# Zejun-Yang/AniPortrait

Hardware: NVIDIA H100
Metric: denoised frames/sec @512x512 L=16 steps=25 (higher is better)
Workload: dtype fp16

## Files before the change

aniportrait_b200/csrc/ap_attention.cu:

```cuda
#include <stdio.h>
#include <stdlib.h>

#include "ap_host.h"
#include "ap_ptx.cuh"
#include "ap_wgmma.cuh"

namespace ap {

__device__ __forceinline__ float fast_exp2(float x) {
  float y;
  asm("ex2.approx.ftz.f32 %0, %1;" : "=f"(y) : "f"(x));
  return y;
}

struct AttnParams {
  int n_frames, tokens, heads, head_dim;
  int bank_tokens;
  int first_bank_frame;
  int frames_per_bank;
  int m_tiles;
  int num_units;
  float scale_log2;
  __half* out;
  long long ldo;
};

template <int DPAD, int BN>
struct AttnCfg {
  static constexpr int SLABS = DPAD / 64;
  static constexpr int Q_BYTES = 128 * DPAD * 2;
  static constexpr int K_BYTES = BN * DPAD * 2;
  static constexpr int KV_STAGE = 2 * K_BYTES;
  static constexpr int BUDGET = 227 * 1024 - 1024 - 256 - Q_BYTES;
  static constexpr int STAGES_RAW = BUDGET / KV_STAGE;
  static constexpr int STAGES = STAGES_RAW > 4 ? 4 : STAGES_RAW;
  static constexpr int SMEM_BYTES = Q_BYTES + STAGES * KV_STAGE + 1024 + 256;
  static_assert(STAGES >= 2, "need at least a double-buffered K/V ring");
  static_assert(DPAD % 64 == 0 && DPAD <= 192 && (BN == 64 || BN == 128), "tile config");
};

template <int DPAD, int BN>
__global__ void __launch_bounds__(384, 1)
attention_kernel(const __grid_constant__ CUtensorMap tmQ, const __grid_constant__ CUtensorMap tmK,
                 const __grid_constant__ CUtensorMap tmV, const __grid_constant__ CUtensorMap tmBK,
                 const __grid_constant__ CUtensorMap tmBV, const AttnParams p) {
  using Cfg = AttnCfg<DPAD, BN>;
  constexpr int ST = Cfg::STAGES;
  griddep_launch_dependents();
  extern __shared__ uint8_t smem_raw[];
  uint8_t* smem = reinterpret_cast<uint8_t*>((reinterpret_cast<uintptr_t>(smem_raw) + 1023) & ~uintptr_t(1023));
  uint8_t* smem_q = smem;
  uint8_t* smem_kv = smem_q + Cfg::Q_BYTES;
  uint64_t* bars = reinterpret_cast<uint64_t*>(smem_kv + ST * Cfg::KV_STAGE);
  uint64_t* q_full = bars + 0;
  uint64_t* q_empty = bars + 1;
  uint64_t* k_full = bars + 2;
  uint64_t* v_full = k_full + ST;
  uint64_t* kv_empty = v_full + ST;

  const int warp = threadIdx.x >> 5;
  const int lane = threadIdx.x & 31;

  if (warp == 0 && lane == 0) {
    tma_prefetch_desc(&tmQ);
    tma_prefetch_desc(&tmK);
    tma_prefetch_desc(&tmV);
    mbar_init(q_full, 1);
    mbar_init(q_empty, 8);
    for (int s = 0; s < ST; ++s) {
      mbar_init(&k_full[s], 1);
      mbar_init(&v_full[s], 1);
      mbar_init(&kv_empty[s], 8);
    }
    fence_mbar_init();
  }
  __syncthreads();
  griddep_wait();

  const int own_tiles = (p.tokens + BN - 1) / BN;
  const int bank_tiles = (p.bank_tokens + BN - 1) / BN;
  const int units_per_frame = p.heads * p.m_tiles;

  auto decode = [&](int unit, int& frame, int& head, int& m_tile, int& T) {
    const int fk = unit / units_per_frame;
    const int rem = unit % units_per_frame;
    frame = (fk + p.first_bank_frame) % p.n_frames;
    head = rem / p.m_tiles;
    m_tile = rem % p.m_tiles;
    const bool has_bank = p.bank_tokens > 0 && frame >= p.first_bank_frame;
    T = own_tiles + (has_bank ? bank_tiles : 0);
  };

  if (warp < 4) {
    setmaxnreg_dec<40>();
    if (warp == 0 && lane == 0) {
      uint32_t g = 0;
      uint32_t uc = 0;
      for (int unit = blockIdx.x; unit < p.num_units; unit += gridDim.x, ++uc) {
        int frame, head, m_tile, T;
        decode(unit, frame, head, m_tile, T);
        mbar_wait_quiet(q_empty, (uc & 1) ^ 1);
        mbar_arrive_expect_tx(q_full, Cfg::Q_BYTES);
#pragma unroll
        for (int s = 0; s < Cfg::SLABS; ++s)
          tma_load_2d(&tmQ, q_full, smem_q + s * (128 * 128), head * DPAD + s * 64, frame * p.tokens + m_tile * 128);
        const int bank_idx = (frame - p.first_bank_frame) / p.frames_per_bank;
        for (int j = 0; j < T; ++j, ++g) {
          const int stage = g % ST;
          const uint32_t ph = (g / ST) & 1;
          mbar_wait_quiet(&kv_empty[stage], ph ^ 1);
          const bool own = j < own_tiles;
          const CUtensorMap* mk = own ? &tmK : &tmBK;
          const CUtensorMap* mv = own ? &tmV : &tmBV;
          const int row = own ? frame * p.tokens + j * BN : bank_idx * p.bank_tokens + (j - own_tiles) * BN;
          uint8_t* kd = smem_kv + stage * Cfg::KV_STAGE;
          uint8_t* vd = kd + Cfg::K_BYTES;
          mbar_arrive_expect_tx(&k_full[stage], Cfg::K_BYTES);
#pragma unroll
          for (int s = 0; s < Cfg::SLABS; ++s)
            tma_load_2d(mk, &k_full[stage], kd + s * (BN * 128), head * DPAD + s * 64, row);
          mbar_arrive_expect_tx(&v_full[stage], Cfg::K_BYTES);
#pragma unroll
          for (int s = 0; s < Cfg::SLABS; ++s)
            tma_load_2d(mv, &v_full[stage], vd + s * (BN * 128), head * DPAD + s * 64, row);
        }
      }
    }
    return;
  }

  setmaxnreg_inc<232>();
  const int wg = (warp >> 2) - 1;
  const int wq = warp & 3;
  const int qd = lane & 3;
  const uint32_t q_base = smem_u32(smem_q) + wg * (64 * 128);
  uint32_t g = 0, uc = 0;
  for (int unit = blockIdx.x; unit < p.num_units; unit += gridDim.x, ++uc) {
    int frame, head, m_tile, T;
    decode(unit, frame, head, m_tile, T);
    float o[DPAD / 2];
#pragma unroll
    for (int i = 0; i < DPAD / 2; ++i) o[i] = 0.f;
    float m_run[2] = {-INFINITY, -INFINITY}, l_run[2] = {0.f, 0.f};
    mbar_wait_quiet(q_full, uc & 1);
    for (int j = 0; j < T; ++j, ++g) {
      const int stage = g % ST;
      const uint32_t ph = (g / ST) & 1;
      const uint32_t k_addr = smem_u32(smem_kv + stage * Cfg::KV_STAGE);
      const uint32_t v_addr = k_addr + Cfg::K_BYTES;
      float s[BN / 2];
      mbar_wait_quiet(&k_full[stage], ph);
      wgmma_fence();
#pragma unroll
      for (int kk = 0; kk < DPAD / 16; ++kk)
        wgmma_ss<BN>(s, wgmma_desc_k_sw128(q_base + (kk / 4) * (128 * 128) + (kk % 4) * 32),
                     wgmma_desc_k_sw128(k_addr + (kk / 4) * (BN * 128) + (kk % 4) * 32), kk != 0);
      wgmma_commit();
      wgmma_wait<0>();
      reg_fence<BN / 2>(s);
      if (j == T - 1) {
        __syncwarp();
        if (lane == 0) mbar_arrive(q_empty);
      }

      const bool own = j < own_tiles;
      const int jj = own ? j : j - own_tiles;
      const int ntok = own ? p.tokens : p.bank_tokens;
      const int valid = min(BN, ntok - jj * BN);
      if (valid != BN) {
#pragma unroll
        for (int i = 0; i < BN / 8; ++i)
#pragma unroll
          for (int e = 0; e < 2; ++e)
            if (8 * i + 2 * qd + e >= valid) {
              s[4 * i + e] = -INFINITY;
              s[4 * i + 2 + e] = -INFINITY;
            }
      }
      float mx[2] = {s[0], s[2]};
#pragma unroll
      for (int i = 0; i < BN / 8; ++i) {
        mx[0] = fmaxf(mx[0], fmaxf(s[4 * i], s[4 * i + 1]));
        mx[1] = fmaxf(mx[1], fmaxf(s[4 * i + 2], s[4 * i + 3]));
      }
      float alpha[2];
#pragma unroll
      for (int r = 0; r < 2; ++r) {
        mx[r] = fmaxf(mx[r], __shfl_xor_sync(0xffffffffu, mx[r], 1));
        mx[r] = fmaxf(mx[r], __shfl_xor_sync(0xffffffffu, mx[r], 2));
        const float m_new = fmaxf(m_run[r], mx[r] * p.scale_log2);
        alpha[r] = fast_exp2(m_run[r] - m_new);
        m_run[r] = m_new;
        l_run[r] *= alpha[r];
      }
#pragma unroll
      for (int i = 0; i < DPAD / 8; ++i) {
        o[4 * i] *= alpha[0]; o[4 * i + 1] *= alpha[0];
        o[4 * i + 2] *= alpha[1]; o[4 * i + 3] *= alpha[1];
      }
      uint32_t pk[BN / 4];
#pragma unroll
      for (int i = 0; i < BN / 8; ++i) {
        const float p0 = fast_exp2(fmaf(s[4 * i], p.scale_log2, -m_run[0]));
        const float p1 = fast_exp2(fmaf(s[4 * i + 1], p.scale_log2, -m_run[0]));
        const float p2 = fast_exp2(fmaf(s[4 * i + 2], p.scale_log2, -m_run[1]));
        const float p3 = fast_exp2(fmaf(s[4 * i + 3], p.scale_log2, -m_run[1]));
        l_run[0] += p0 + p1;
        l_run[1] += p2 + p3;
        const __half2 h01 = __floats2half2_rn(p0, p1), h23 = __floats2half2_rn(p2, p3);
        pk[2 * i] = *reinterpret_cast<const uint32_t*>(&h01);
        pk[2 * i + 1] = *reinterpret_cast<const uint32_t*>(&h23);
      }
      mbar_wait_quiet(&v_full[stage], ph);
      wgmma_fence();
#pragma unroll
      for (int kk = 0; kk < BN / 16; ++kk)
        wgmma_rs_tb<DPAD>(o, pk + 4 * kk, wgmma_desc_mn_sw128(v_addr + kk * (16 * 128), BN * 128), 1);
      wgmma_commit();
      wgmma_wait<0>();
      reg_fence<DPAD / 2>(o);
      __syncwarp();
      if (lane == 0) mbar_arrive(&kv_empty[stage]);
    }
#pragma unroll
    for (int r = 0; r < 2; ++r) {
      l_run[r] += __shfl_xor_sync(0xffffffffu, l_run[r], 1);
      l_run[r] += __shfl_xor_sync(0xffffffffu, l_run[r], 2);
    }
#pragma unroll
    for (int r = 0; r < 2; ++r) {
      const float inv_l = 1.f / l_run[r];
      const int q_idx = m_tile * 128 + wg * 64 + wq * 16 + (lane >> 2) + 8 * r;
      if (q_idx < p.tokens) {
        __half* dst = p.out + ((long long)frame * p.tokens + q_idx) * p.ldo + head * p.head_dim;
#pragma unroll
        for (int i = 0; i < DPAD / 8; ++i)
          if (8 * i + 2 * qd < p.head_dim)
            *reinterpret_cast<__half2*>(dst + 8 * i + 2 * qd) =
                __floats2half2_rn(o[4 * i + 2 * r] * inv_l, o[4 * i + 2 * r + 1] * inv_l);
      }
    }
  }
}

template <int DPAD, int BN>
static int launch_attention(const CUtensorMap* maps, const AttnParams& p, cudaStream_t stream) {
  using Cfg = AttnCfg<DPAD, BN>;
  static bool attr_set = false;
  if (!attr_set) {
    AP_CHECK_CUDA(cudaFuncSetAttribute(attention_kernel<DPAD, BN>, cudaFuncAttributeMaxDynamicSharedMemorySize,
                                       Cfg::SMEM_BYTES));
    attr_set = true;
  }
  const int grid = p.num_units < num_sms() ? p.num_units : num_sms();
  AP_LAUNCH((attention_kernel<DPAD, BN>), grid, 384, Cfg::SMEM_BYTES, stream, maps[0], maps[1], maps[2], maps[3], maps[4], p);
  AP_CHECK_CUDA(cudaGetLastError());
  return AP_OK;
}

}

using namespace ap;

extern "C" int ap_attention_f16(const void* q, const void* k, const void* v, long long ld_qkv, const void* bank_k,
                                const void* bank_v, long long ld_bank, int bank_tokens, int n_banks, int n_frames,
                                int tokens, int heads, int head_dim, int dpad, int first_bank_frame,
                                int frames_per_bank, float scale, void* out, long long ldo, void* stream) {
  AP_REQUIRE(q && k && v && out, "attention: null pointer");
  AP_REQUIRE(dpad == 64 || dpad == 128 || dpad == 192, "attention: dpad must be 64/128/192 (got %d)", dpad);
  AP_REQUIRE(head_dim % 8 == 0 && head_dim <= dpad, "attention: head_dim %d must be a multiple of 8 and <= dpad", head_dim);
  AP_REQUIRE(ld_qkv % 8 == 0 && ldo % 8 == 0, "attention: leading dims must be multiples of 8 elements");
  AP_REQUIRE(n_frames > 0 && tokens > 0 && heads > 0, "attention: bad shape");
  const bool has_bank = bank_k != nullptr && bank_tokens > 0;
  AP_REQUIRE(!has_bank || (bank_v && frames_per_bank > 0 && first_bank_frame >= 0 && n_banks > 0),
             "attention: bad bank arguments");
  const int bn = dpad == 192 ? 64 : 128;
  AttnParams p{};
  p.n_frames = n_frames;
  p.tokens = tokens;
  p.heads = heads;
  p.head_dim = head_dim;
  p.bank_tokens = has_bank ? bank_tokens : 0;
  p.first_bank_frame = has_bank ? first_bank_frame : 0;
  p.frames_per_bank = has_bank ? frames_per_bank : 1;
  p.m_tiles = (tokens + 127) / 128;
  p.num_units = n_frames * heads * p.m_tiles;
  p.scale_log2 = scale * 1.4426950408889634f;
  p.out = (__half*)out;
  p.ldo = ldo;
  if (has_bank) {
    const int max_bank = (n_frames - 1 - first_bank_frame) / frames_per_bank;
    AP_REQUIRE(first_bank_frame >= n_frames || max_bank < n_banks, "attention: bank index out of range");
  }

  CUtensorMap maps[5];
  const uint64_t cols = (uint64_t)heads * dpad;
  auto mk = [&](CUtensorMap* tm, const void* base, uint64_t rows, long long ld, uint32_t box_rows) -> int {
    const uint64_t dims[2] = {cols, rows};
    const uint64_t strides[1] = {(uint64_t)ld * 2};
    const uint32_t box[2] = {64, box_rows};
    return encode_tmap(tm, base, 2, dims, strides, box, true);
  };
  int rc;
  const uint64_t rows = (uint64_t)n_frames * tokens;
  if ((rc = mk(&maps[0], q, rows, ld_qkv, 128))) return rc;
  if ((rc = mk(&maps[1], k, rows, ld_qkv, bn))) return rc;
  if ((rc = mk(&maps[2], v, rows, ld_qkv, bn))) return rc;
  if (has_bank) {
    const uint64_t brows = (uint64_t)n_banks * bank_tokens;
    if ((rc = mk(&maps[3], bank_k, brows, ld_bank, bn))) return rc;
    if ((rc = mk(&maps[4], bank_v, brows, ld_bank, bn))) return rc;
  } else {
    maps[3] = maps[1];
    maps[4] = maps[2];
  }
  cudaStream_t st = (cudaStream_t)stream;
  if (dpad == 64) return launch_attention<64, 128>(maps, p, st);
  if (dpad == 128) return launch_attention<128, 128>(maps, p, st);
  return launch_attention<192, 64>(maps, p, st);
}
```

aniportrait_b200/csrc/ap_ptx.cuh:

```cuda
#pragma once
#include <cuda.h>
#include <cuda_fp16.h>
#include <cuda_runtime.h>
#include <stdint.h>
#include <stdio.h>

namespace ap {

__device__ __forceinline__ void griddep_launch_dependents() { asm volatile("griddepcontrol.launch_dependents;" ::: "memory"); }
__device__ __forceinline__ void griddep_wait() { asm volatile("griddepcontrol.wait;" ::: "memory"); }

__device__ __forceinline__ float gelu_erf(float x) {
  const float z = fminf(fabsf(x) * 0.70710678118654752f, 4.3f);
  float q = fmaf(1.686094986e-05f, z, -4.376256625e-04f);
  q = fmaf(q, z, 4.960034474e-03f);
  q = fmaf(q, z, -3.321249048e-02f);
  q = fmaf(q, z, 1.515097036e-01f);
  q = fmaf(q, z, 9.176268788e-01f);
  q = fmaf(q, z, 1.627959694e+00f);
  float e;
  asm("ex2.approx.ftz.f32 %0, %1;" : "=f"(e) : "f"(-q * z));
  return fmaxf(x, 0.f) - z * 0.70710678118654752f * e;
}

__device__ __forceinline__ uint32_t smem_u32(const void* p) {
  return static_cast<uint32_t>(__cvta_generic_to_shared(p));
}

__device__ __forceinline__ uint32_t elect_one() {
  uint32_t pred = 0;
  asm volatile(
      "{\n\t"
      ".reg .pred P1;\n\t"
      "elect.sync _|P1, 0xffffffff;\n\t"
      "selp.u32 %0, 1, 0, P1;\n\t"
      "}\n"
      : "=r"(pred));
  return pred;
}

__device__ __forceinline__ void mbar_init(uint64_t* bar, uint32_t count) {
  asm volatile("mbarrier.init.shared::cta.b64 [%0], %1;" ::"r"(smem_u32(bar)), "r"(count) : "memory");
}
__device__ __forceinline__ void fence_mbar_init() {
  asm volatile("fence.mbarrier_init.release.cluster;" ::: "memory");
}
__device__ __forceinline__ void fence_proxy_async_smem() {
  asm volatile("fence.proxy.async.shared::cta;" ::: "memory");
}
__device__ __forceinline__ void mbar_arrive_expect_tx(uint64_t* bar, uint32_t bytes) {
  asm volatile("mbarrier.arrive.expect_tx.shared::cta.b64 _, [%0], %1;" ::"r"(smem_u32(bar)), "r"(bytes)
               : "memory");
}
__device__ __forceinline__ void mbar_arrive(uint64_t* bar) {
  asm volatile("mbarrier.arrive.shared::cta.b64 _, [%0];" ::"r"(smem_u32(bar)) : "memory");
}
__device__ __forceinline__ uint32_t mbar_try_wait(uint64_t* bar, uint32_t parity) {
  uint32_t done;
  asm volatile(
      "{\n\t"
      ".reg .pred P1;\n\t"
      "mbarrier.try_wait.parity.shared::cta.b64 P1, [%1], %2;\n\t"
      "selp.u32 %0, 1, 0, P1;\n\t"
      "}\n"
      : "=r"(done)
      : "r"(smem_u32(bar)), "r"(parity)
      : "memory");
  return done;
}
#ifndef AP_MBAR_TIMEOUT_CYCLES
#define AP_MBAR_TIMEOUT_CYCLES (8000000000ll)
#endif
__device__ __forceinline__ void mbar_wait(uint64_t* bar, uint32_t parity) {
  if (mbar_try_wait(bar, parity)) return;
  long long t0 = clock64();
  while (!mbar_try_wait(bar, parity)) {
    if (clock64() - t0 > AP_MBAR_TIMEOUT_CYCLES) {
      printf("ap: mbarrier timeout block=(%d,%d) thread=%d bar=0x%x parity=%u\n", blockIdx.x, blockIdx.y, threadIdx.x,
             smem_u32(bar), parity);
      __trap();
    }
  }
}

__device__ __forceinline__ void mbar_wait_quiet(uint64_t* bar, uint32_t parity) {
  if (mbar_try_wait(bar, parity)) return;
  long long t0 = clock64();
  while (!mbar_try_wait(bar, parity))
    if (clock64() - t0 > AP_MBAR_TIMEOUT_CYCLES) __trap();
}

__device__ __forceinline__ void tma_prefetch_desc(const CUtensorMap* m) {
  asm volatile("prefetch.tensormap [%0];" ::"l"(reinterpret_cast<uint64_t>(m)) : "memory");
}
__device__ __forceinline__ void tma_load_2d(const CUtensorMap* m, uint64_t* bar, void* dst, int c0, int c1) {
  asm volatile(
      "cp.async.bulk.tensor.2d.shared::cluster.global.mbarrier::complete_tx::bytes [%0], [%1, {%3, %4}], [%2];" ::"r"(
          smem_u32(dst)),
      "l"(reinterpret_cast<uint64_t>(m)), "r"(smem_u32(bar)), "r"(c0), "r"(c1)
      : "memory");
}
__device__ __forceinline__ void tma_load_3d(const CUtensorMap* m, uint64_t* bar, void* dst, int c0, int c1, int c2) {
  asm volatile(
      "cp.async.bulk.tensor.3d.shared::cluster.global.mbarrier::complete_tx::bytes [%0], [%1, {%3, %4, %5}], [%2];" ::
          "r"(smem_u32(dst)),
      "l"(reinterpret_cast<uint64_t>(m)), "r"(smem_u32(bar)), "r"(c0), "r"(c1), "r"(c2)
      : "memory");
}
__device__ __forceinline__ void tma_load_4d(const CUtensorMap* m, uint64_t* bar, void* dst, int c0, int c1, int c2,
                                            int c3) {
  asm volatile(
      "cp.async.bulk.tensor.4d.shared::cluster.global.mbarrier::complete_tx::bytes [%0], [%1, {%3, %4, %5, %6}], "
      "[%2];" ::"r"(smem_u32(dst)),
      "l"(reinterpret_cast<uint64_t>(m)), "r"(smem_u32(bar)), "r"(c0), "r"(c1), "r"(c2), "r"(c3)
      : "memory");
}
__device__ __forceinline__ void tma_load_5d(const CUtensorMap* m, uint64_t* bar, void* dst, int c0, int c1, int c2,
                                            int c3, int c4) {
  asm volatile(
      "cp.async.bulk.tensor.5d.shared::cluster.global.mbarrier::complete_tx::bytes [%0], [%1, {%3, %4, %5, %6, %7}], "
      "[%2];" ::"r"(smem_u32(dst)),
      "l"(reinterpret_cast<uint64_t>(m)), "r"(smem_u32(bar)), "r"(c0), "r"(c1), "r"(c2), "r"(c3), "r"(c4)
      : "memory");
}

__device__ __forceinline__ void tma_store_2d(const CUtensorMap* m, const void* src, int c0, int c1) {
  asm volatile("cp.async.bulk.tensor.2d.global.shared::cta.bulk_group [%0, {%2, %3}], [%1];" ::"l"(
                   reinterpret_cast<uint64_t>(m)),
               "r"(smem_u32(src)), "r"(c0), "r"(c1)
               : "memory");
}
__device__ __forceinline__ void tma_store_4d(const CUtensorMap* m, const void* src, int c0, int c1, int c2, int c3) {
  asm volatile("cp.async.bulk.tensor.4d.global.shared::cta.bulk_group [%0, {%2, %3, %4, %5}], [%1];" ::"l"(
                   reinterpret_cast<uint64_t>(m)),
               "r"(smem_u32(src)), "r"(c0), "r"(c1), "r"(c2), "r"(c3)
               : "memory");
}
__device__ __forceinline__ void tma_store_commit() { asm volatile("cp.async.bulk.commit_group;" ::: "memory"); }
template <int N>
__device__ __forceinline__ void tma_store_wait_read() {
  asm volatile("cp.async.bulk.wait_group.read %0;" ::"n"(N) : "memory");
}
template <int N>
__device__ __forceinline__ void tma_store_wait_all() {
  asm volatile("cp.async.bulk.wait_group %0;" ::"n"(N) : "memory");
}

__device__ __forceinline__ void wgmma_fence() { asm volatile("wgmma.fence.sync.aligned;" ::: "memory"); }
__device__ __forceinline__ void wgmma_commit() { asm volatile("wgmma.commit_group.sync.aligned;" ::: "memory"); }
template <int N>
__device__ __forceinline__ void wgmma_wait() {
  asm volatile("wgmma.wait_group.sync.aligned %0;" ::"n"(N) : "memory");
}
template <int N>
__device__ __forceinline__ void reg_fence(float* r) {
#pragma unroll
  for (int i = 0; i < N; ++i) asm volatile("" : "+f"(r[i])::"memory");
}
template <uint32_t kRegs>
__device__ __forceinline__ void setmaxnreg_inc() { asm volatile("setmaxnreg.inc.sync.aligned.u32 %0;" ::"n"(kRegs)); }
template <uint32_t kRegs>
__device__ __forceinline__ void setmaxnreg_dec() { asm volatile("setmaxnreg.dec.sync.aligned.u32 %0;" ::"n"(kRegs)); }

__device__ __forceinline__ uint64_t wgmma_desc_k_sw128(uint32_t smem_addr) {
  uint64_t d = 0;
  d |= static_cast<uint64_t>((smem_addr >> 4) & 0x3FFF);
  d |= static_cast<uint64_t>(1) << 16;
  d |= static_cast<uint64_t>(1024 >> 4) << 32;
  d |= static_cast<uint64_t>(1) << 62;
  return d;
}
__device__ __forceinline__ uint64_t wgmma_desc_mn_sw128(uint32_t smem_addr, uint32_t lbo_bytes) {
  uint64_t d = 0;
  d |= static_cast<uint64_t>((smem_addr >> 4) & 0x3FFF);
  d |= static_cast<uint64_t>((lbo_bytes >> 4) & 0x3FFF) << 16;
  d |= static_cast<uint64_t>(1024 >> 4) << 32;
  d |= static_cast<uint64_t>(1) << 62;
  return d;
}

__device__ __forceinline__ void named_bar_sync(uint32_t id, uint32_t nthreads) {
  asm volatile("bar.sync %0, %1;" ::"r"(id), "r"(nthreads) : "memory");
}

}
```

aniportrait_b200/csrc/ap_wgmma.cuh:

```cuda
#pragma once
#include <stdint.h>

namespace ap {

template <int N>
__device__ __forceinline__ void wgmma_ss(float* d, uint64_t da, uint64_t db, uint32_t scale_d);
template <int N>
__device__ __forceinline__ void wgmma_rs_tb(float* d, const uint32_t* a, uint64_t db, uint32_t scale_d);

template <>
__device__ __forceinline__ void wgmma_ss<32>(float* d, uint64_t da, uint64_t db, uint32_t scale_d) {
  asm volatile(
      "{\n\t.reg .pred p;\n\tsetp.ne.b32 p, %18, 0;\n\t"
      "wgmma.mma_async.sync.aligned.m64n32k16.f32.f16.f16 {%0, %1, %2, %3, %4, %5, %6, %7, %8, %9, %10, %11, %12, %13, %14, %15}, %16, %17, p, 1, 1, 0, 0;\n\t}\n"
      : "+f"(d[0]), "+f"(d[1]), "+f"(d[2]), "+f"(d[3]), "+f"(d[4]), "+f"(d[5]), "+f"(d[6]), "+f"(d[7]), "+f"(d[8]), "+f"(d[9]), "+f"(d[10]), "+f"(d[11]), "+f"(d[12]), "+f"(d[13]), "+f"(d[14]), "+f"(d[15])
      : "l"(da), "l"(db), "r"(scale_d));
}
template <>
__device__ __forceinline__ void wgmma_ss<64>(float* d, uint64_t da, uint64_t db, uint32_t scale_d) {
  asm volatile(
      "{\n\t.reg .pred p;\n\tsetp.ne.b32 p, %34, 0;\n\t"
      "wgmma.mma_async.sync.aligned.m64n64k16.f32.f16.f16 {%0, %1, %2, %3, %4, %5, %6, %7, %8, %9, %10, %11, %12, %13, %14, %15, %16, %17, %18, %19, %20, %21, %22, %23, %24, %25, %26, %27, %28, %29, %30, %31}, %32, %33, p, 1, 1, 0, 0;\n\t}\n"
      : "+f"(d[0]), "+f"(d[1]), "+f"(d[2]), "+f"(d[3]), "+f"(d[4]), "+f"(d[5]), "+f"(d[6]), "+f"(d[7]), "+f"(d[8]), "+f"(d[9]), "+f"(d[10]), "+f"(d[11]), "+f"(d[12]), "+f"(d[13]), "+f"(d[14]), "+f"(d[15]), "+f"(d[16]), "+f"(d[17]), "+f"(d[18]), "+f"(d[19]), "+f"(d[20]), "+f"(d[21]), "+f"(d[22]), "+f"(d[23]), "+f"(d[24]), "+f"(d[25]), "+f"(d[26]), "+f"(d[27]), "+f"(d[28]), "+f"(d[29]), "+f"(d[30]), "+f"(d[31])
      : "l"(da), "l"(db), "r"(scale_d));
}
template <>
__device__ __forceinline__ void wgmma_ss<128>(float* d, uint64_t da, uint64_t db, uint32_t scale_d) {
  asm volatile(
      "{\n\t.reg .pred p;\n\tsetp.ne.b32 p, %66, 0;\n\t"
      "wgmma.mma_async.sync.aligned.m64n128k16.f32.f16.f16 {%0, %1, %2, %3, %4, %5, %6, %7, %8, %9, %10, %11, %12, %13, %14, %15, %16, %17, %18, %19, %20, %21, %22, %23, %24, %25, %26, %27, %28, %29, %30, %31, %32, %33, %34, %35, %36, %37, %38, %39, %40, %41, %42, %43, %44, %45, %46, %47, %48, %49, %50, %51, %52, %53, %54, %55, %56, %57, %58, %59, %60, %61, %62, %63}, %64, %65, p, 1, 1, 0, 0;\n\t}\n"
      : "+f"(d[0]), "+f"(d[1]), "+f"(d[2]), "+f"(d[3]), "+f"(d[4]), "+f"(d[5]), "+f"(d[6]), "+f"(d[7]), "+f"(d[8]), "+f"(d[9]), "+f"(d[10]), "+f"(d[11]), "+f"(d[12]), "+f"(d[13]), "+f"(d[14]), "+f"(d[15]), "+f"(d[16]), "+f"(d[17]), "+f"(d[18]), "+f"(d[19]), "+f"(d[20]), "+f"(d[21]), "+f"(d[22]), "+f"(d[23]), "+f"(d[24]), "+f"(d[25]), "+f"(d[26]), "+f"(d[27]), "+f"(d[28]), "+f"(d[29]), "+f"(d[30]), "+f"(d[31]), "+f"(d[32]), "+f"(d[33]), "+f"(d[34]), "+f"(d[35]), "+f"(d[36]), "+f"(d[37]), "+f"(d[38]), "+f"(d[39]), "+f"(d[40]), "+f"(d[41]), "+f"(d[42]), "+f"(d[43]), "+f"(d[44]), "+f"(d[45]), "+f"(d[46]), "+f"(d[47]), "+f"(d[48]), "+f"(d[49]), "+f"(d[50]), "+f"(d[51]), "+f"(d[52]), "+f"(d[53]), "+f"(d[54]), "+f"(d[55]), "+f"(d[56]), "+f"(d[57]), "+f"(d[58]), "+f"(d[59]), "+f"(d[60]), "+f"(d[61]), "+f"(d[62]), "+f"(d[63])
      : "l"(da), "l"(db), "r"(scale_d));
}
template <>
__device__ __forceinline__ void wgmma_ss<160>(float* d, uint64_t da, uint64_t db, uint32_t scale_d) {
  asm volatile(
      "{\n\t.reg .pred p;\n\tsetp.ne.b32 p, %82, 0;\n\t"
      "wgmma.mma_async.sync.aligned.m64n160k16.f32.f16.f16 {%0, %1, %2, %3, %4, %5, %6, %7, %8, %9, %10, %11, %12, %13, %14, %15, %16, %17, %18, %19, %20, %21, %22, %23, %24, %25, %26, %27, %28, %29, %30, %31, %32, %33, %34, %35, %36, %37, %38, %39, %40, %41, %42, %43, %44, %45, %46, %47, %48, %49, %50, %51, %52, %53, %54, %55, %56, %57, %58, %59, %60, %61, %62, %63, %64, %65, %66, %67, %68, %69, %70, %71, %72, %73, %74, %75, %76, %77, %78, %79}, %80, %81, p, 1, 1, 0, 0;\n\t}\n"
      : "+f"(d[0]), "+f"(d[1]), "+f"(d[2]), "+f"(d[3]), "+f"(d[4]), "+f"(d[5]), "+f"(d[6]), "+f"(d[7]), "+f"(d[8]), "+f"(d[9]), "+f"(d[10]), "+f"(d[11]), "+f"(d[12]), "+f"(d[13]), "+f"(d[14]), "+f"(d[15]), "+f"(d[16]), "+f"(d[17]), "+f"(d[18]), "+f"(d[19]), "+f"(d[20]), "+f"(d[21]), "+f"(d[22]), "+f"(d[23]), "+f"(d[24]), "+f"(d[25]), "+f"(d[26]), "+f"(d[27]), "+f"(d[28]), "+f"(d[29]), "+f"(d[30]), "+f"(d[31]), "+f"(d[32]), "+f"(d[33]), "+f"(d[34]), "+f"(d[35]), "+f"(d[36]), "+f"(d[37]), "+f"(d[38]), "+f"(d[39]), "+f"(d[40]), "+f"(d[41]), "+f"(d[42]), "+f"(d[43]), "+f"(d[44]), "+f"(d[45]), "+f"(d[46]), "+f"(d[47]), "+f"(d[48]), "+f"(d[49]), "+f"(d[50]), "+f"(d[51]), "+f"(d[52]), "+f"(d[53]), "+f"(d[54]), "+f"(d[55]), "+f"(d[56]), "+f"(d[57]), "+f"(d[58]), "+f"(d[59]), "+f"(d[60]), "+f"(d[61]), "+f"(d[62]), "+f"(d[63]), "+f"(d[64]), "+f"(d[65]), "+f"(d[66]), "+f"(d[67]), "+f"(d[68]), "+f"(d[69]), "+f"(d[70]), "+f"(d[71]), "+f"(d[72]), "+f"(d[73]), "+f"(d[74]), "+f"(d[75]), "+f"(d[76]), "+f"(d[77]), "+f"(d[78]), "+f"(d[79])
      : "l"(da), "l"(db), "r"(scale_d));
}
template <>
__device__ __forceinline__ void wgmma_ss<256>(float* d, uint64_t da, uint64_t db, uint32_t scale_d) {
  asm volatile(
      "{\n\t.reg .pred p;\n\tsetp.ne.b32 p, %130, 0;\n\t"
      "wgmma.mma_async.sync.aligned.m64n256k16.f32.f16.f16 {%0, %1, %2, %3, %4, %5, %6, %7, %8, %9, %10, %11, %12, %13, %14, %15, %16, %17, %18, %19, %20, %21, %22, %23, %24, %25, %26, %27, %28, %29, %30, %31, %32, %33, %34, %35, %36, %37, %38, %39, %40, %41, %42, %43, %44, %45, %46, %47, %48, %49, %50, %51, %52, %53, %54, %55, %56, %57, %58, %59, %60, %61, %62, %63, %64, %65, %66, %67, %68, %69, %70, %71, %72, %73, %74, %75, %76, %77, %78, %79, %80, %81, %82, %83, %84, %85, %86, %87, %88, %89, %90, %91, %92, %93, %94, %95, %96, %97, %98, %99, %100, %101, %102, %103, %104, %105, %106, %107, %108, %109, %110, %111, %112, %113, %114, %115, %116, %117, %118, %119, %120, %121, %122, %123, %124, %125, %126, %127}, %128, %129, p, 1, 1, 0, 0;\n\t}\n"
      : "+f"(d[0]), "+f"(d[1]), "+f"(d[2]), "+f"(d[3]), "+f"(d[4]), "+f"(d[5]), "+f"(d[6]), "+f"(d[7]), "+f"(d[8]), "+f"(d[9]), "+f"(d[10]), "+f"(d[11]), "+f"(d[12]), "+f"(d[13]), "+f"(d[14]), "+f"(d[15]), "+f"(d[16]), "+f"(d[17]), "+f"(d[18]), "+f"(d[19]), "+f"(d[20]), "+f"(d[21]), "+f"(d[22]), "+f"(d[23]), "+f"(d[24]), "+f"(d[25]), "+f"(d[26]), "+f"(d[27]), "+f"(d[28]), "+f"(d[29]), "+f"(d[30]), "+f"(d[31]), "+f"(d[32]), "+f"(d[33]), "+f"(d[34]), "+f"(d[35]), "+f"(d[36]), "+f"(d[37]), "+f"(d[38]), "+f"(d[39]), "+f"(d[40]), "+f"(d[41]), "+f"(d[42]), "+f"(d[43]), "+f"(d[44]), "+f"(d[45]), "+f"(d[46]), "+f"(d[47]), "+f"(d[48]), "+f"(d[49]), "+f"(d[50]), "+f"(d[51]), "+f"(d[52]), "+f"(d[53]), "+f"(d[54]), "+f"(d[55]), "+f"(d[56]), "+f"(d[57]), "+f"(d[58]), "+f"(d[59]), "+f"(d[60]), "+f"(d[61]), "+f"(d[62]), "+f"(d[63]), "+f"(d[64]), "+f"(d[65]), "+f"(d[66]), "+f"(d[67]), "+f"(d[68]), "+f"(d[69]), "+f"(d[70]), "+f"(d[71]), "+f"(d[72]), "+f"(d[73]), "+f"(d[74]), "+f"(d[75]), "+f"(d[76]), "+f"(d[77]), "+f"(d[78]), "+f"(d[79]), "+f"(d[80]), "+f"(d[81]), "+f"(d[82]), "+f"(d[83]), "+f"(d[84]), "+f"(d[85]), "+f"(d[86]), "+f"(d[87]), "+f"(d[88]), "+f"(d[89]), "+f"(d[90]), "+f"(d[91]), "+f"(d[92]), "+f"(d[93]), "+f"(d[94]), "+f"(d[95]), "+f"(d[96]), "+f"(d[97]), "+f"(d[98]), "+f"(d[99]), "+f"(d[100]), "+f"(d[101]), "+f"(d[102]), "+f"(d[103]), "+f"(d[104]), "+f"(d[105]), "+f"(d[106]), "+f"(d[107]), "+f"(d[108]), "+f"(d[109]), "+f"(d[110]), "+f"(d[111]), "+f"(d[112]), "+f"(d[113]), "+f"(d[114]), "+f"(d[115]), "+f"(d[116]), "+f"(d[117]), "+f"(d[118]), "+f"(d[119]), "+f"(d[120]), "+f"(d[121]), "+f"(d[122]), "+f"(d[123]), "+f"(d[124]), "+f"(d[125]), "+f"(d[126]), "+f"(d[127])
      : "l"(da), "l"(db), "r"(scale_d));
}
template <>
__device__ __forceinline__ void wgmma_rs_tb<64>(float* d, const uint32_t* a, uint64_t db, uint32_t scale_d) {
  asm volatile(
      "{\n\t.reg .pred p;\n\tsetp.ne.b32 p, %37, 0;\n\t"
      "wgmma.mma_async.sync.aligned.m64n64k16.f32.f16.f16 {%0, %1, %2, %3, %4, %5, %6, %7, %8, %9, %10, %11, %12, %13, %14, %15, %16, %17, %18, %19, %20, %21, %22, %23, %24, %25, %26, %27, %28, %29, %30, %31}, {%32, %33, %34, %35}, %36, p, 1, 1, 1;\n\t}\n"
      : "+f"(d[0]), "+f"(d[1]), "+f"(d[2]), "+f"(d[3]), "+f"(d[4]), "+f"(d[5]), "+f"(d[6]), "+f"(d[7]), "+f"(d[8]), "+f"(d[9]), "+f"(d[10]), "+f"(d[11]), "+f"(d[12]), "+f"(d[13]), "+f"(d[14]), "+f"(d[15]), "+f"(d[16]), "+f"(d[17]), "+f"(d[18]), "+f"(d[19]), "+f"(d[20]), "+f"(d[21]), "+f"(d[22]), "+f"(d[23]), "+f"(d[24]), "+f"(d[25]), "+f"(d[26]), "+f"(d[27]), "+f"(d[28]), "+f"(d[29]), "+f"(d[30]), "+f"(d[31])
      : "r"(a[0]), "r"(a[1]), "r"(a[2]), "r"(a[3]), "l"(db), "r"(scale_d));
}
template <>
__device__ __forceinline__ void wgmma_rs_tb<128>(float* d, const uint32_t* a, uint64_t db, uint32_t scale_d) {
  asm volatile(
      "{\n\t.reg .pred p;\n\tsetp.ne.b32 p, %69, 0;\n\t"
      "wgmma.mma_async.sync.aligned.m64n128k16.f32.f16.f16 {%0, %1, %2, %3, %4, %5, %6, %7, %8, %9, %10, %11, %12, %13, %14, %15, %16, %17, %18, %19, %20, %21, %22, %23, %24, %25, %26, %27, %28, %29, %30, %31, %32, %33, %34, %35, %36, %37, %38, %39, %40, %41, %42, %43, %44, %45, %46, %47, %48, %49, %50, %51, %52, %53, %54, %55, %56, %57, %58, %59, %60, %61, %62, %63}, {%64, %65, %66, %67}, %68, p, 1, 1, 1;\n\t}\n"
      : "+f"(d[0]), "+f"(d[1]), "+f"(d[2]), "+f"(d[3]), "+f"(d[4]), "+f"(d[5]), "+f"(d[6]), "+f"(d[7]), "+f"(d[8]), "+f"(d[9]), "+f"(d[10]), "+f"(d[11]), "+f"(d[12]), "+f"(d[13]), "+f"(d[14]), "+f"(d[15]), "+f"(d[16]), "+f"(d[17]), "+f"(d[18]), "+f"(d[19]), "+f"(d[20]), "+f"(d[21]), "+f"(d[22]), "+f"(d[23]), "+f"(d[24]), "+f"(d[25]), "+f"(d[26]), "+f"(d[27]), "+f"(d[28]), "+f"(d[29]), "+f"(d[30]), "+f"(d[31]), "+f"(d[32]), "+f"(d[33]), "+f"(d[34]), "+f"(d[35]), "+f"(d[36]), "+f"(d[37]), "+f"(d[38]), "+f"(d[39]), "+f"(d[40]), "+f"(d[41]), "+f"(d[42]), "+f"(d[43]), "+f"(d[44]), "+f"(d[45]), "+f"(d[46]), "+f"(d[47]), "+f"(d[48]), "+f"(d[49]), "+f"(d[50]), "+f"(d[51]), "+f"(d[52]), "+f"(d[53]), "+f"(d[54]), "+f"(d[55]), "+f"(d[56]), "+f"(d[57]), "+f"(d[58]), "+f"(d[59]), "+f"(d[60]), "+f"(d[61]), "+f"(d[62]), "+f"(d[63])
      : "r"(a[0]), "r"(a[1]), "r"(a[2]), "r"(a[3]), "l"(db), "r"(scale_d));
}
template <>
__device__ __forceinline__ void wgmma_rs_tb<192>(float* d, const uint32_t* a, uint64_t db, uint32_t scale_d) {
  asm volatile(
      "{\n\t.reg .pred p;\n\tsetp.ne.b32 p, %101, 0;\n\t"
      "wgmma.mma_async.sync.aligned.m64n192k16.f32.f16.f16 {%0, %1, %2, %3, %4, %5, %6, %7, %8, %9, %10, %11, %12, %13, %14, %15, %16, %17, %18, %19, %20, %21, %22, %23, %24, %25, %26, %27, %28, %29, %30, %31, %32, %33, %34, %35, %36, %37, %38, %39, %40, %41, %42, %43, %44, %45, %46, %47, %48, %49, %50, %51, %52, %53, %54, %55, %56, %57, %58, %59, %60, %61, %62, %63, %64, %65, %66, %67, %68, %69, %70, %71, %72, %73, %74, %75, %76, %77, %78, %79, %80, %81, %82, %83, %84, %85, %86, %87, %88, %89, %90, %91, %92, %93, %94, %95}, {%96, %97, %98, %99}, %100, p, 1, 1, 1;\n\t}\n"
      : "+f"(d[0]), "+f"(d[1]), "+f"(d[2]), "+f"(d[3]), "+f"(d[4]), "+f"(d[5]), "+f"(d[6]), "+f"(d[7]), "+f"(d[8]), "+f"(d[9]), "+f"(d[10]), "+f"(d[11]), "+f"(d[12]), "+f"(d[13]), "+f"(d[14]), "+f"(d[15]), "+f"(d[16]), "+f"(d[17]), "+f"(d[18]), "+f"(d[19]), "+f"(d[20]), "+f"(d[21]), "+f"(d[22]), "+f"(d[23]), "+f"(d[24]), "+f"(d[25]), "+f"(d[26]), "+f"(d[27]), "+f"(d[28]), "+f"(d[29]), "+f"(d[30]), "+f"(d[31]), "+f"(d[32]), "+f"(d[33]), "+f"(d[34]), "+f"(d[35]), "+f"(d[36]), "+f"(d[37]), "+f"(d[38]), "+f"(d[39]), "+f"(d[40]), "+f"(d[41]), "+f"(d[42]), "+f"(d[43]), "+f"(d[44]), "+f"(d[45]), "+f"(d[46]), "+f"(d[47]), "+f"(d[48]), "+f"(d[49]), "+f"(d[50]), "+f"(d[51]), "+f"(d[52]), "+f"(d[53]), "+f"(d[54]), "+f"(d[55]), "+f"(d[56]), "+f"(d[57]), "+f"(d[58]), "+f"(d[59]), "+f"(d[60]), "+f"(d[61]), "+f"(d[62]), "+f"(d[63]), "+f"(d[64]), "+f"(d[65]), "+f"(d[66]), "+f"(d[67]), "+f"(d[68]), "+f"(d[69]), "+f"(d[70]), "+f"(d[71]), "+f"(d[72]), "+f"(d[73]), "+f"(d[74]), "+f"(d[75]), "+f"(d[76]), "+f"(d[77]), "+f"(d[78]), "+f"(d[79]), "+f"(d[80]), "+f"(d[81]), "+f"(d[82]), "+f"(d[83]), "+f"(d[84]), "+f"(d[85]), "+f"(d[86]), "+f"(d[87]), "+f"(d[88]), "+f"(d[89]), "+f"(d[90]), "+f"(d[91]), "+f"(d[92]), "+f"(d[93]), "+f"(d[94]), "+f"(d[95])
      : "r"(a[0]), "r"(a[1]), "r"(a[2]), "r"(a[3]), "l"(db), "r"(scale_d));
}

}
```

Measured before the change: 5.601.

## Pipeline QK/PV wgmma in attention, add 3-consumer mode and exact head-dim tiles

Restructures the attention consumer loop so the QK^T wgmma for tile j is issued together with the PV wgmma for tile j-1, overlapping softmax with tensor-core work. For small head dims it uses three consumer warpgroups (192-row Q tiles) with rebalanced register allocation. The kernel is now templated on the head dim rounded up to 16 rather than padded to 64, which cuts wasted MMA work. It also computes some exponentials with a cubic polynomial on FMA units to offload the MUFU unit. Risks include register pressure with the extra live accumulators, lower polynomial precision, and more template instantiations.

After: 5.766, median of 6. 2.9% higher.

```diff
diff --git a/aniportrait_b200/csrc/ap_attention.cu b/aniportrait_b200/csrc/ap_attention.cu
--- a/aniportrait_b200/csrc/ap_attention.cu
+++ b/aniportrait_b200/csrc/ap_attention.cu
@@ -15,6 +15,7 @@
 
 struct AttnParams {
   int n_frames, tokens, heads, head_dim;
+  int dpad;
   int bank_tokens;
   int first_bank_frame;
   int frames_per_bank;
@@ -25,10 +26,26 @@
   long long ldo;
 };
 
-template <int DPAD, int BN>
+#ifndef AP_ATTN_POLY_OF_16
+#define AP_ATTN_POLY_OF_16 2
+#endif
+constexpr int POLY_OF_16 = AP_ATTN_POLY_OF_16;
+
+template <int DH>
+struct AttnKeyTile {
+  static constexpr int value = DH > 128 ? 64 : 128;
+};
+
+#ifndef AP_ATTN_NC3_MAX_DH
+#define AP_ATTN_NC3_MAX_DH 64
+#endif
+__host__ __device__ constexpr int attn_consumers(int dh) { return dh <= AP_ATTN_NC3_MAX_DH ? 3 : 2; }
+
+template <int DPAD, int BN, int NC>
 struct AttnCfg {
   static constexpr int SLABS = DPAD / 64;
-  static constexpr int Q_BYTES = 128 * DPAD * 2;
+  static constexpr int Q_ROWS = 64 * NC;
+  static constexpr int Q_BYTES = Q_ROWS * DPAD * 2;
   static constexpr int K_BYTES = BN * DPAD * 2;
   static constexpr int KV_STAGE = 2 * K_BYTES;
   static constexpr int BUDGET = 227 * 1024 - 1024 - 256 - Q_BYTES;
@@ -39,12 +56,16 @@
   static_assert(DPAD % 64 == 0 && DPAD <= 192 && (BN == 64 || BN == 128), "tile config");
 };
 
-template <int DPAD, int BN>
-__global__ void __launch_bounds__(384, 1)
+template <int DH>
+__global__ void __launch_bounds__(128 * (1 + attn_consumers(DH)), 1)
 attention_kernel(const __grid_constant__ CUtensorMap tmQ, const __grid_constant__ CUtensorMap tmK,
                  const __grid_constant__ CUtensorMap tmV, const __grid_constant__ CUtensorMap tmBK,
                  const __grid_constant__ CUtensorMap tmBV, const AttnParams p) {
-  using Cfg = AttnCfg<DPAD, BN>;
+  constexpr int DPAD = (DH + 63) / 64 * 64;
+  constexpr int BN = AttnKeyTile<DH>::value;
+  constexpr int NC = attn_consumers(DH);
+  using Cfg = AttnCfg<DPAD, BN, NC>;
+  static_assert(DH % 16 == 0, "head dim step");
   constexpr int ST = Cfg::STAGES;
   griddep_launch_dependents();
   extern __shared__ uint8_t smem_raw[];
@@ -66,11 +87,11 @@
     tma_prefetch_desc(&tmK);
     tma_prefetch_desc(&tmV);
     mbar_init(q_full, 1);
-    mbar_init(q_empty, 8);
+    mbar_init(q_empty, 4 * NC);
     for (int s = 0; s < ST; ++s) {
       mbar_init(&k_full[s], 1);
       mbar_init(&v_full[s], 1);
-      mbar_init(&kv_empty[s], 8);
+      mbar_init(&kv_empty[s], 4 * NC);
     }
     fence_mbar_init();
   }
@@ -92,7 +113,7 @@
   };
 
   if (warp < 4) {
-    setmaxnreg_dec<40>();
+    setmaxnreg_dec<NC == 3 ? 24 : 40>();
     if (warp == 0 && lane == 0) {
       uint32_t g = 0;
       uint32_t uc = 0;
@@ -103,7 +124,8 @@
         mbar_arrive_expect_tx(q_full, Cfg::Q_BYTES);
 #pragma unroll
         for (int s = 0; s < Cfg::SLABS; ++s)
-          tma_load_2d(&tmQ, q_full, smem_q + s * (128 * 128), head * DPAD + s * 64, frame * p.tokens + m_tile * 128);
+          tma_load_2d(&tmQ, q_full, smem_q + s * (Cfg::Q_ROWS * 128), head * p.dpad + s * 64,
+                      frame * p.tokens + m_tile * Cfg::Q_ROWS);
         const int bank_idx = (frame - p.first_bank_frame) / p.frames_per_bank;
         for (int j = 0; j < T; ++j, ++g) {
           const int stage = g % ST;
@@ -118,110 +140,149 @@
           mbar_arrive_expect_tx(&k_full[stage], Cfg::K_BYTES);
 #pragma unroll
           for (int s = 0; s < Cfg::SLABS; ++s)
-            tma_load_2d(mk, &k_full[stage], kd + s * (BN * 128), head * DPAD + s * 64, row);
+            tma_load_2d(mk, &k_full[stage], kd + s * (BN * 128), head * p.dpad + s * 64, row);
           mbar_arrive_expect_tx(&v_full[stage], Cfg::K_BYTES);
 #pragma unroll
           for (int s = 0; s < Cfg::SLABS; ++s)
-            tma_load_2d(mv, &v_full[stage], vd + s * (BN * 128), head * DPAD + s * 64, row);
+            tma_load_2d(mv, &v_full[stage], vd + s * (BN * 128), head * p.dpad + s * 64, row);
         }
       }
     }
     return;
   }
 
-  setmaxnreg_inc<232>();
+  setmaxnreg_inc<NC == 3 ? 160 : 232>();
   const int wg = (warp >> 2) - 1;
   const int wq = warp & 3;
   const int qd = lane & 3;
   const uint32_t q_base = smem_u32(smem_q) + wg * (64 * 128);
+
+  auto k_smem = [&](uint32_t t) { return smem_u32(smem_kv + (t % ST) * Cfg::KV_STAGE); };
+  auto issue_qk = [&](float* s, uint32_t k_addr) {
+#pragma unroll
+    for (int kk = 0; kk < DH / 16; ++kk)
+      wgmma_ss<BN>(s, wgmma_desc_k_sw128(q_base + (kk / 4) * (Cfg::Q_ROWS * 128) + (kk % 4) * 32),
+                   wgmma_desc_k_sw128(k_addr + (kk / 4) * (BN * 128) + (kk % 4) * 32), kk != 0);
+  };
+  auto issue_pv = [&](float* o, const uint32_t* pk, uint32_t v_addr) {
+#pragma unroll
+    for (int kk = 0; kk < BN / 16; ++kk)
+      wgmma_rs_tb<DH>(o, pk + 4 * kk, wgmma_desc_mn_sw128(v_addr + kk * (16 * 128), BN * 128), 1);
+  };
+  auto softmax = [&](float* s, int j, int own_tiles, float* m_run, float* l_run, float* alpha) {
+    const bool own = j < own_tiles;
+    const int jj = own ? j : j - own_tiles;
+    const int ntok = own ? p.tokens : p.bank_tokens;
+    const int valid = min(BN, ntok - jj * BN);
+    if (valid != BN) {
+#pragma unroll
+      for (int i = 0; i < BN / 8; ++i)
+#pragma unroll
+        for (int e = 0; e < 2; ++e)
+          if (8 * i + 2 * qd + e >= valid) {
+            s[4 * i + e] = -INFINITY;
+            s[4 * i + 2 + e] = -INFINITY;
+          }
+    }
+    float mx[2] = {s[0], s[2]};
+#pragma unroll
+    for (int i = 0; i < BN / 8; ++i) {
+      mx[0] = fmaxf(mx[0], fmaxf(s[4 * i], s[4 * i + 1]));
+      mx[1] = fmaxf(mx[1], fmaxf(s[4 * i + 2], s[4 * i + 3]));
+    }
+#pragma unroll
+    for (int r = 0; r < 2; ++r) {
+      mx[r] = fmaxf(mx[r], __shfl_xor_sync(0xffffffffu, mx[r], 1));
+      mx[r] = fmaxf(mx[r], __shfl_xor_sync(0xffffffffu, mx[r], 2));
+      const float m_new = fmaxf(m_run[r], mx[r] * p.scale_log2);
+      alpha[r] = fast_exp2(m_run[r] - m_new);
+      m_run[r] = m_new;
+      l_run[r] *= alpha[r];
+    }
+#pragma unroll
+    for (int i = 0; i < BN / 8; ++i) {
+#pragma unroll
+      for (int e = 0; e < 4; ++e) {
+        const float x = fmaf(s[4 * i + e], p.scale_log2, -m_run[e >> 1]);
+        s[4 * i + e] = (4 * i + e) % 16 < POLY_OF_16 ? exp2_poly3(x) : fast_exp2(x);
+      }
+      l_run[0] += s[4 * i] + s[4 * i + 1];
+      l_run[1] += s[4 * i + 2] + s[4 * i + 3];
+    }
+  };
+  auto pack = [&](const float* s, uint32_t* pk) {
+#pragma unroll
+    for (int i = 0; i < BN / 8; ++i) {
+      const __half2 h01 = __floats2half2_rn(s[4 * i], s[4 * i + 1]), h23 = __floats2half2_rn(s[4 * i + 2], s[4 * i + 3]);
+      pk[2 * i] = *reinterpret_cast<const uint32_t*>(&h01);
+      pk[2 * i + 1] = *reinterpret_cast<const uint32_t*>(&h23);
+    }
+  };
+  auto release_q = [&]() {
+    __syncwarp();
+    if (lane == 0) mbar_arrive(q_empty);
+  };
+  auto release_kv = [&](uint32_t t) {
+    __syncwarp();
+    if (lane == 0) mbar_arrive(&kv_empty[t % ST]);
+  };
+
   uint32_t g = 0, uc = 0;
   for (int unit = blockIdx.x; unit < p.num_units; unit += gridDim.x, ++uc) {
     int frame, head, m_tile, T;
     decode(unit, frame, head, m_tile, T);
-    float o[DPAD / 2];
-#pragma unroll
-    for (int i = 0; i < DPAD / 2; ++i) o[i] = 0.f;
-    float m_run[2] = {-INFINITY, -INFINITY}, l_run[2] = {0.f, 0.f};
+    float o[DH / 2];
+#pragma unroll
+    for (int i = 0; i < DH / 2; ++i) o[i] = 0.f;
+    float m_run[2] = {-INFINITY, -INFINITY}, l_run[2] = {0.f, 0.f}, alpha[2];
+    float s[BN / 2];
+    uint32_t pk[BN / 4];
     mbar_wait_quiet(q_full, uc & 1);
-    for (int j = 0; j < T; ++j, ++g) {
-      const int stage = g % ST;
-      const uint32_t ph = (g / ST) & 1;
-      const uint32_t k_addr = smem_u32(smem_kv + stage * Cfg::KV_STAGE);
-      const uint32_t v_addr = k_addr + Cfg::K_BYTES;
-      float s[BN / 2];
-      mbar_wait_quiet(&k_full[stage], ph);
+
+    mbar_wait_quiet(&k_full[g % ST], (g / ST) & 1);
+    wgmma_fence();
+    issue_qk(s, k_smem(g));
+    wgmma_commit();
+    wgmma_wait<0>();
+    reg_fence<BN / 2>(s);
+    if (T == 1) release_q();
+    softmax(s, 0, own_tiles, m_run, l_run, alpha);
+    pack(s, pk);
+
+    for (int j = 1; j < T; ++j) {
+      const uint32_t t = g + j;
+      mbar_wait_quiet(&k_full[t % ST], (t / ST) & 1);
+      mbar_wait_quiet(&v_full[(t - 1) % ST], ((t - 1) / ST) & 1);
       wgmma_fence();
-#pragma unroll
-      for (int kk = 0; kk < DPAD / 16; ++kk)
-        wgmma_ss<BN>(s, wgmma_desc_k_sw128(q_base + (kk / 4) * (128 * 128) + (kk % 4) * 32),
-                     wgmma_desc_k_sw128(k_addr + (kk / 4) * (BN * 128) + (kk % 4) * 32), kk != 0);
+      issue_qk(s, k_smem(t));
       wgmma_commit();
+      issue_pv(o, pk, k_smem(t - 1) + Cfg::K_BYTES);
+      wgmma_commit();
+      wgmma_wait<1>();
+      reg_fence<BN / 2>(s);
+      if (j == T - 1) release_q();
+      softmax(s, j, own_tiles, m_run, l_run, alpha);
       wgmma_wait<0>();
+      reg_fence<DH / 2>(o);
       reg_fence<BN / 2>(s);
-      if (j == T - 1) {
-        __syncwarp();
-        if (lane == 0) mbar_arrive(q_empty);
-      }
-
-      const bool own = j < own_tiles;
-      const int jj = own ? j : j - own_tiles;
-      const int ntok = own ? p.tokens : p.bank_tokens;
-      const int valid = min(BN, ntok - jj * BN);
-      if (valid != BN) {
-#pragma unroll
-        for (int i = 0; i < BN / 8; ++i)
-#pragma unroll
-          for (int e = 0; e < 2; ++e)
-            if (8 * i + 2 * qd + e >= valid) {
-              s[4 * i + e] = -INFINITY;
-              s[4 * i + 2 + e] = -INFINITY;
-            }
-      }
-      float mx[2] = {s[0], s[2]};
-#pragma unroll
-      for (int i = 0; i < BN / 8; ++i) {
-        mx[0] = fmaxf(mx[0], fmaxf(s[4 * i], s[4 * i + 1]));
-        mx[1] = fmaxf(mx[1], fmaxf(s[4 * i + 2], s[4 * i + 3]));
-      }
-      float alpha[2];
-#pragma unroll
-      for (int r = 0; r < 2; ++r) {
-        mx[r] = fmaxf(mx[r], __shfl_xor_sync(0xffffffffu, mx[r], 1));
-        mx[r] = fmaxf(mx[r], __shfl_xor_sync(0xffffffffu, mx[r], 2));
-        const float m_new = fmaxf(m_run[r], mx[r] * p.scale_log2);
-        alpha[r] = fast_exp2(m_run[r] - m_new);
-        m_run[r] = m_new;
-        l_run[r] *= alpha[r];
-      }
-#pragma unroll
-      for (int i = 0; i < DPAD / 8; ++i) {
+      release_kv(t - 1);
+#pragma unroll
+      for (int i = 0; i < DH / 8; ++i) {
         o[4 * i] *= alpha[0]; o[4 * i + 1] *= alpha[0];
         o[4 * i + 2] *= alpha[1]; o[4 * i + 3] *= alpha[1];
       }
-      uint32_t pk[BN / 4];
-#pragma unroll
-      for (int i = 0; i < BN / 8; ++i) {
-        const float p0 = fast_exp2(fmaf(s[4 * i], p.scale_log2, -m_run[0]));
-        const float p1 = fast_exp2(fmaf(s[4 * i + 1], p.scale_log2, -m_run[0]));
-        const float p2 = fast_exp2(fmaf(s[4 * i + 2], p.scale_log2, -m_run[1]));
-        const float p3 = fast_exp2(fmaf(s[4 * i + 3], p.scale_log2, -m_run[1]));
-        l_run[0] += p0 + p1;
-        l_run[1] += p2 + p3;
-        const __half2 h01 = __floats2half2_rn(p0, p1), h23 = __floats2half2_rn(p2, p3);
-        pk[2 * i] = *reinterpret_cast<const uint32_t*>(&h01);
-        pk[2 * i + 1] = *reinterpret_cast<const uint32_t*>(&h23);
-      }
-      mbar_wait_quiet(&v_full[stage], ph);
-      wgmma_fence();
-#pragma unroll
-      for (int kk = 0; kk < BN / 16; ++kk)
-        wgmma_rs_tb<DPAD>(o, pk + 4 * kk, wgmma_desc_mn_sw128(v_addr + kk * (16 * 128), BN * 128), 1);
-      wgmma_commit();
-      wgmma_wait<0>();
-      reg_fence<DPAD / 2>(o);
-      __syncwarp();
-      if (lane == 0) mbar_arrive(&kv_empty[stage]);
-    }
+      pack(s, pk);
+    }
+    const uint32_t t_last = g + T - 1;
+    mbar_wait_quiet(&v_full[t_last % ST], (t_last / ST) & 1);
+    wgmma_fence();
+    issue_pv(o, pk, k_smem(t_last) + Cfg::K_BYTES);
+    wgmma_commit();
+    wgmma_wait<0>();
+    reg_fence<DH / 2>(o);
+    release_kv(t_last);
+    g += T;
+
 #pragma unroll
     for (int r = 0; r < 2; ++r) {
       l_run[r] += __shfl_xor_sync(0xffffffffu, l_run[r], 1);
@@ -230,11 +291,11 @@
 #pragma unroll
     for (int r = 0; r < 2; ++r) {
       const float inv_l = 1.f / l_run[r];
-      const int q_idx = m_tile * 128 + wg * 64 + wq * 16 + (lane >> 2) + 8 * r;
+      const int q_idx = m_tile * Cfg::Q_ROWS + wg * 64 + wq * 16 + (lane >> 2) + 8 * r;
       if (q_idx < p.tokens) {
         __half* dst = p.out + ((long long)frame * p.tokens + q_idx) * p.ldo + head * p.head_dim;
 #pragma unroll
-        for (int i = 0; i < DPAD / 8; ++i)
+        for (int i = 0; i < DH / 8; ++i)
           if (8 * i + 2 * qd < p.head_dim)
             *reinterpret_cast<__half2*>(dst + 8 * i + 2 * qd) =
                 __floats2half2_rn(o[4 * i + 2 * r] * inv_l, o[4 * i + 2 * r + 1] * inv_l);
@@ -243,17 +304,18 @@
   }
 }
 
-template <int DPAD, int BN>
+template <int DH>
 static int launch_attention(const CUtensorMap* maps, const AttnParams& p, cudaStream_t stream) {
-  using Cfg = AttnCfg<DPAD, BN>;
+  using Cfg = AttnCfg<(DH + 63) / 64 * 64, AttnKeyTile<DH>::value, attn_consumers(DH)>;
   static bool attr_set = false;
   if (!attr_set) {
-    AP_CHECK_CUDA(cudaFuncSetAttribute(attention_kernel<DPAD, BN>, cudaFuncAttributeMaxDynamicSharedMemorySize,
+    AP_CHECK_CUDA(cudaFuncSetAttribute(attention_kernel<DH>, cudaFuncAttributeMaxDynamicSharedMemorySize,
                                        Cfg::SMEM_BYTES));
     attr_set = true;
   }
   const int grid = p.num_units < num_sms() ? p.num_units : num_sms();
-  AP_LAUNCH((attention_kernel<DPAD, BN>), grid, 384, Cfg::SMEM_BYTES, stream, maps[0], maps[1], maps[2], maps[3], maps[4], p);
+  AP_LAUNCH((attention_kernel<DH>), grid, 128 * (1 + attn_consumers(DH)), Cfg::SMEM_BYTES, stream, maps[0], maps[1], maps[2], maps[3],
+            maps[4], p);
   AP_CHECK_CUDA(cudaGetLastError());
   return AP_OK;
 }
@@ -274,16 +336,19 @@
   const bool has_bank = bank_k != nullptr && bank_tokens > 0;
   AP_REQUIRE(!has_bank || (bank_v && frames_per_bank > 0 && first_bank_frame >= 0 && n_banks > 0),
              "attention: bad bank arguments");
-  const int bn = dpad == 192 ? 64 : 128;
+  const int dh = (head_dim + 15) / 16 * 16;
+  const int bn = dh > 128 ? 64 : 128;
   AttnParams p{};
   p.n_frames = n_frames;
   p.tokens = tokens;
   p.heads = heads;
   p.head_dim = head_dim;
+  p.dpad = dpad;
   p.bank_tokens = has_bank ? bank_tokens : 0;
   p.first_bank_frame = has_bank ? first_bank_frame : 0;
   p.frames_per_bank = has_bank ? frames_per_bank : 1;
-  p.m_tiles = (tokens + 127) / 128;
+  const int q_rows = 64 * attn_consumers(dh);
+  p.m_tiles = (tokens + q_rows - 1) / q_rows;
   p.num_units = n_frames * heads * p.m_tiles;
   p.scale_log2 = scale * 1.4426950408889634f;
   p.out = (__half*)out;
@@ -303,7 +368,7 @@
   };
   int rc;
   const uint64_t rows = (uint64_t)n_frames * tokens;
-  if ((rc = mk(&maps[0], q, rows, ld_qkv, 128))) return rc;
+  if ((rc = mk(&maps[0], q, rows, ld_qkv, q_rows))) return rc;
   if ((rc = mk(&maps[1], k, rows, ld_qkv, bn))) return rc;
   if ((rc = mk(&maps[2], v, rows, ld_qkv, bn))) return rc;
   if (has_bank) {
@@ -315,7 +380,18 @@
     maps[4] = maps[2];
   }
   cudaStream_t st = (cudaStream_t)stream;
-  if (dpad == 64) return launch_attention<64, 128>(maps, p, st);
-  if (dpad == 128) return launch_attention<128, 128>(maps, p, st);
-  return launch_attention<192, 64>(maps, p, st);
-}
+  switch (dh / 16) {
+    case 1: return launch_attention<16>(maps, p, st);
+    case 2: return launch_attention<32>(maps, p, st);
+    case 3: return launch_attention<48>(maps, p, st);
+    case 4: return launch_attention<64>(maps, p, st);
+    case 5: return launch_attention<80>(maps, p, st);
+    case 6: return launch_attention<96>(maps, p, st);
+    case 7: return launch_attention<112>(maps, p, st);
+    case 8: return launch_attention<128>(maps, p, st);
+    case 9: return launch_attention<144>(maps, p, st);
+    case 10: return launch_attention<160>(maps, p, st);
+    case 11: return launch_attention<176>(maps, p, st);
+    default: return launch_attention<192>(maps, p, st);
+  }
+}
diff --git a/aniportrait_b200/csrc/ap_ptx.cuh b/aniportrait_b200/csrc/ap_ptx.cuh
--- a/aniportrait_b200/csrc/ap_ptx.cuh
+++ b/aniportrait_b200/csrc/ap_ptx.cuh
@@ -21,6 +21,19 @@
   float e;
   asm("ex2.approx.ftz.f32 %0, %1;" : "=f"(e) : "f"(-q * z));
   return fmaxf(x, 0.f) - z * 0.70710678118654752f * e;
+}
+
+__device__ __forceinline__ float exp2_poly3(float x) {
+  x = fmaxf(x, -127.f);
+  const float j = x + 12582912.f;
+  const float f = x - (j - 12582912.f);
+  float p = fmaf(5.517167031e-02f, f, 2.426111252e-01f);
+  p = fmaf(p, f, 6.932609853e-01f);
+  p = fmaf(p, f, 9.999280730e-01f);
+  const float scale = __uint_as_float((__float_as_uint(j) << 23) + 0x3F800000u);
+  float r;
+  asm("mul.ftz.f32 %0, %1, %2;" : "=f"(r) : "f"(p), "f"(scale));
+  return r;
 }
 
 __device__ __forceinline__ uint32_t smem_u32(const void* p) {
diff --git a/aniportrait_b200/csrc/ap_wgmma.cuh b/aniportrait_b200/csrc/ap_wgmma.cuh
--- a/aniportrait_b200/csrc/ap_wgmma.cuh
+++ b/aniportrait_b200/csrc/ap_wgmma.cuh
@@ -49,6 +49,30 @@
       : "l"(da), "l"(db), "r"(scale_d));
 }
 template <>
+__device__ __forceinline__ void wgmma_rs_tb<16>(float* d, const uint32_t* a, uint64_t db, uint32_t scale_d) {
+  asm volatile(
+      "{\n\t.reg .pred p;\n\tsetp.ne.b32 p, %13, 0;\n\t"
+      "wgmma.mma_async.sync.aligned.m64n16k16.f32.f16.f16 {%0, %1, %2, %3, %4, %5, %6, %7}, {%8, %9, %10, %11}, %12, p, 1, 1, 1;\n\t}\n"
+      : "+f"(d[0]), "+f"(d[1]), "+f"(d[2]), "+f"(d[3]), "+f"(d[4]), "+f"(d[5]), "+f"(d[6]), "+f"(d[7])
+      : "r"(a[0]), "r"(a[1]), "r"(a[2]), "r"(a[3]), "l"(db), "r"(scale_d));
+}
+template <>
+__device__ __forceinline__ void wgmma_rs_tb<32>(float* d, const uint32_t* a, uint64_t db, uint32_t scale_d) {
+  asm volatile(
+      "{\n\t.reg .pred p;\n\tsetp.ne.b32 p, %21, 0;\n\t"
+      "wgmma.mma_async.sync.aligned.m64n32k16.f32.f16.f16 {%0, %1, %2, %3, %4, %5, %6, %7, %8, %9, %10, %11, %12, %13, %14, %15}, {%16, %17, %18, %19}, %20, p, 1, 1, 1;\n\t}\n"
+      : "+f"(d[0]), "+f"(d[1]), "+f"(d[2]), "+f"(d[3]), "+f"(d[4]), "+f"(d[5]), "+f"(d[6]), "+f"(d[7]), "+f"(d[8]), "+f"(d[9]), "+f"(d[10]), "+f"(d[11]), "+f"(d[12]), "+f"(d[13]), "+f"(d[14]), "+f"(d[15])
+      : "r"(a[0]), "r"(a[1]), "r"(a[2]), "r"(a[3]), "l"(db), "r"(scale_d));
+}
+template <>
+__device__ __forceinline__ void wgmma_rs_tb<48>(float* d, const uint32_t* a, uint64_t db, uint32_t scale_d) {
+  asm volatile(
+      "{\n\t.reg .pred p;\n\tsetp.ne.b32 p, %29, 0;\n\t"
+      "wgmma.mma_async.sync.aligned.m64n48k16.f32.f16.f16 {%0, %1, %2, %3, %4, %5, %6, %7, %8, %9, %10, %11, %12, %13, %14, %15, %16, %17, %18, %19, %20, %21, %22, %23}, {%24, %25, %26, %27}, %28, p, 1, 1, 1;\n\t}\n"
+      : "+f"(d[0]), "+f"(d[1]), "+f"(d[2]), "+f"(d[3]), "+f"(d[4]), "+f"(d[5]), "+f"(d[6]), "+f"(d[7]), "+f"(d[8]), "+f"(d[9]), "+f"(d[10]), "+f"(d[11]), "+f"(d[12]), "+f"(d[13]), "+f"(d[14]), "+f"(d[15]), "+f"(d[16]), "+f"(d[17]), "+f"(d[18]), "+f"(d[19]), "+f"(d[20]), "+f"(d[21]), "+f"(d[22]), "+f"(d[23])
+      : "r"(a[0]), "r"(a[1]), "r"(a[2]), "r"(a[3]), "l"(db), "r"(scale_d));
+}
+template <>
 __device__ __forceinline__ void wgmma_rs_tb<64>(float* d, const uint32_t* a, uint64_t db, uint32_t scale_d) {
   asm volatile(
       "{\n\t.reg .pred p;\n\tsetp.ne.b32 p, %37, 0;\n\t"
@@ -57,11 +81,59 @@
       : "r"(a[0]), "r"(a[1]), "r"(a[2]), "r"(a[3]), "l"(db), "r"(scale_d));
 }
 template <>
+__device__ __forceinline__ void wgmma_rs_tb<80>(float* d, const uint32_t* a, uint64_t db, uint32_t scale_d) {
+  asm volatile(
+      "{\n\t.reg .pred p;\n\tsetp.ne.b32 p, %45, 0;\n\t"
+      "wgmma.mma_async.sync.aligned.m64n80k16.f32.f16.f16 {%0, %1, %2, %3, %4, %5, %6, %7, %8, %9, %10, %11, %12, %13, %14, %15, %16, %17, %18, %19, %20, %21, %22, %23, %24, %25, %26, %27, %28, %29, %30, %31, %32, %33, %34, %35, %36, %37, %38, %39}, {%40, %41, %42, %43}, %44, p, 1, 1, 1;\n\t}\n"
+      : "+f"(d[0]), "+f"(d[1]), "+f"(d[2]), "+f"(d[3]), "+f"(d[4]), "+f"(d[5]), "+f"(d[6]), "+f"(d[7]), "+f"(d[8]), "+f"(d[9]), "+f"(d[10]), "+f"(d[11]), "+f"(d[12]), "+f"(d[13]), "+f"(d[14]), "+f"(d[15]), "+f"(d[16]), "+f"(d[17]), "+f"(d[18]), "+f"(d[19]), "+f"(d[20]), "+f"(d[21]), "+f"(d[22]), "+f"(d[23]), "+f"(d[24]), "+f"(d[25]), "+f"(d[26]), "+f"(d[27]), "+f"(d[28]), "+f"(d[29]), "+f"(d[30]), "+f"(d[31]), "+f"(d[32]), "+f"(d[33]), "+f"(d[34]), "+f"(d[35]), "+f"(d[36]), "+f"(d[37]), "+f"(d[38]), "+f"(d[39])
+      : "r"(a[0]), "r"(a[1]), "r"(a[2]), "r"(a[3]), "l"(db), "r"(scale_d));
+}
+template <>
+__device__ __forceinline__ void wgmma_rs_tb<96>(float* d, const uint32_t* a, uint64_t db, uint32_t scale_d) {
+  asm volatile(
+      "{\n\t.reg .pred p;\n\tsetp.ne.b32 p, %53, 0;\n\t"
+      "wgmma.mma_async.sync.aligned.m64n96k16.f32.f16.f16 {%0, %1, %2, %3, %4, %5, %6, %7, %8, %9, %10, %11, %12, %13, %14, %15, %16, %17, %18, %19, %20, %21, %22, %23, %24, %25, %26, %27, %28, %29, %30, %31, %32, %33, %34, %35, %36, %37, %38, %39, %40, %41, %42, %43, %44, %45, %46, %47}, {%48, %49, %50, %51}, %52, p, 1, 1, 1;\n\t}\n"
+      : "+f"(d[0]), "+f"(d[1]), "+f"(d[2]), "+f"(d[3]), "+f"(d[4]), "+f"(d[5]), "+f"(d[6]), "+f"(d[7]), "+f"(d[8]), "+f"(d[9]), "+f"(d[10]), "+f"(d[11]), "+f"(d[12]), "+f"(d[13]), "+f"(d[14]), "+f"(d[15]), "+f"(d[16]), "+f"(d[17]), "+f"(d[18]), "+f"(d[19]), "+f"(d[20]), "+f"(d[21]), "+f"(d[22]), "+f"(d[23]), "+f"(d[24]), "+f"(d[25]), "+f"(d[26]), "+f"(d[27]), "+f"(d[28]), "+f"(d[29]), "+f"(d[30]), "+f"(d[31]), "+f"(d[32]), "+f"(d[33]), "+f"(d[34]), "+f"(d[35]), "+f"(d[36]), "+f"(d[37]), "+f"(d[38]), "+f"(d[39]), "+f"(d[40]), "+f"(d[41]), "+f"(d[42]), "+f"(d[43]), "+f"(d[44]), "+f"(d[45]), "+f"(d[46]), "+f"(d[47])
+      : "r"(a[0]), "r"(a[1]), "r"(a[2]), "r"(a[3]), "l"(db), "r"(scale_d));
+}
+template <>
+__device__ __forceinline__ void wgmma_rs_tb<112>(float* d, const uint32_t* a, uint64_t db, uint32_t scale_d) {
+  asm volatile(
+      "{\n\t.reg .pred p;\n\tsetp.ne.b32 p, %61, 0;\n\t"
+      "wgmma.mma_async.sync.aligned.m64n112k16.f32.f16.f16 {%0, %1, %2, %3, %4, %5, %6, %7, %8, %9, %10, %11, %12, %13, %14, %15, %16, %17, %18, %19, %20, %21, %22, %23, %24, %25, %26, %27, %28, %29, %30, %31, %32, %33, %34, %35, %36, %37, %38, %39, %40, %41, %42, %43, %44, %45, %46, %47, %48, %49, %50, %51, %52, %53, %54, %55}, {%56, %57, %58, %59}, %60, p, 1, 1, 1;\n\t}\n"
+      : "+f"(d[0]), "+f"(d[1]), "+f"(d[2]), "+f"(d[3]), "+f"(d[4]), "+f"(d[5]), "+f"(d[6]), "+f"(d[7]), "+f"(d[8]), "+f"(d[9]), "+f"(d[10]), "+f"(d[11]), "+f"(d[12]), "+f"(d[13]), "+f"(d[14]), "+f"(d[15]), "+f"(d[16]), "+f"(d[17]), "+f"(d[18]), "+f"(d[19]), "+f"(d[20]), "+f"(d[21]), "+f"(d[22]), "+f"(d[23]), "+f"(d[24]), "+f"(d[25]), "+f"(d[26]), "+f"(d[27]), "+f"(d[28]), "+f"(d[29]), "+f"(d[30]), "+f"(d[31]), "+f"(d[32]), "+f"(d[33]), "+f"(d[34]), "+f"(d[35]), "+f"(d[36]), "+f"(d[37]), "+f"(d[38]), "+f"(d[39]), "+f"(d[40]), "+f"(d[41]), "+f"(d[42]), "+f"(d[43]), "+f"(d[44]), "+f"(d[45]), "+f"(d[46]), "+f"(d[47]), "+f"(d[48]), "+f"(d[49]), "+f"(d[50]), "+f"(d[51]), "+f"(d[52]), "+f"(d[53]), "+f"(d[54]), "+f"(d[55])
+      : "r"(a[0]), "r"(a[1]), "r"(a[2]), "r"(a[3]), "l"(db), "r"(scale_d));
+}
+template <>
 __device__ __forceinline__ void wgmma_rs_tb<128>(float* d, const uint32_t* a, uint64_t db, uint32_t scale_d) {
   asm volatile(
       "{\n\t.reg .pred p;\n\tsetp.ne.b32 p, %69, 0;\n\t"
       "wgmma.mma_async.sync.aligned.m64n128k16.f32.f16.f16 {%0, %1, %2, %3, %4, %5, %6, %7, %8, %9, %10, %11, %12, %13, %14, %15, %16, %17, %18, %19, %20, %21, %22, %23, %24, %25, %26, %27, %28, %29, %30, %31, %32, %33, %34, %35, %36, %37, %38, %39, %40, %41, %42, %43, %44, %45, %46, %47, %48, %49, %50, %51, %52, %53, %54, %55, %56, %57, %58, %59, %60, %61, %62, %63}, {%64, %65, %66, %67}, %68, p, 1, 1, 1;\n\t}\n"
       : "+f"(d[0]), "+f"(d[1]), "+f"(d[2]), "+f"(d[3]), "+f"(d[4]), "+f"(d[5]), "+f"(d[6]), "+f"(d[7]), "+f"(d[8]), "+f"(d[9]), "+f"(d[10]), "+f"(d[11]), "+f"(d[12]), "+f"(d[13]), "+f"(d[14]), "+f"(d[15]), "+f"(d[16]), "+f"(d[17]), "+f"(d[18]), "+f"(d[19]), "+f"(d[20]), "+f"(d[21]), "+f"(d[22]), "+f"(d[23]), "+f"(d[24]), "+f"(d[25]), "+f"(d[26]), "+f"(d[27]), "+f"(d[28]), "+f"(d[29]), "+f"(d[30]), "+f"(d[31]), "+f"(d[32]), "+f"(d[33]), "+f"(d[34]), "+f"(d[35]), "+f"(d[36]), "+f"(d[37]), "+f"(d[38]), "+f"(d[39]), "+f"(d[40]), "+f"(d[41]), "+f"(d[42]), "+f"(d[43]), "+f"(d[44]), "+f"(d[45]), "+f"(d[46]), "+f"(d[47]), "+f"(d[48]), "+f"(d[49]), "+f"(d[50]), "+f"(d[51]), "+f"(d[52]), "+f"(d[53]), "+f"(d[54]), "+f"(d[55]), "+f"(d[56]), "+f"(d[57]), "+f"(d[58]), "+f"(d[59]), "+f"(d[60]), "+f"(d[61]), "+f"(d[62]), "+f"(d[63])
+      : "r"(a[0]), "r"(a[1]), "r"(a[2]), "r"(a[3]), "l"(db), "r"(scale_d));
+}
+template <>
+__device__ __forceinline__ void wgmma_rs_tb<144>(float* d, const uint32_t* a, uint64_t db, uint32_t scale_d) {
+  asm volatile(
+      "{\n\t.reg .pred p;\n\tsetp.ne.b32 p, %77, 0;\n\t"
+      "wgmma.mma_async.sync.aligned.m64n144k16.f32.f16.f16 {%0, %1, %2, %3, %4, %5, %6, %7, %8, %9, %10, %11, %12, %13, %14, %15, %16, %17, %18, %19, %20, %21, %22, %23, %24, %25, %26, %27, %28, %29, %30, %31, %32, %33, %34, %35, %36, %37, %38, %39, %40, %41, %42, %43, %44, %45, %46, %47, %48, %49, %50, %51, %52, %53, %54, %55, %56, %57, %58, %59, %60, %61, %62, %63, %64, %65, %66, %67, %68, %69, %70, %71}, {%72, %73, %74, %75}, %76, p, 1, 1, 1;\n\t}\n"
+      : "+f"(d[0]), "+f"(d[1]), "+f"(d[2]), "+f"(d[3]), "+f"(d[4]), "+f"(d[5]), "+f"(d[6]), "+f"(d[7]), "+f"(d[8]), "+f"(d[9]), "+f"(d[10]), "+f"(d[11]), "+f"(d[12]), "+f"(d[13]), "+f"(d[14]), "+f"(d[15]), "+f"(d[16]), "+f"(d[17]), "+f"(d[18]), "+f"(d[19]), "+f"(d[20]), "+f"(d[21]), "+f"(d[22]), "+f"(d[23]), "+f"(d[24]), "+f"(d[25]), "+f"(d[26]), "+f"(d[27]), "+f"(d[28]), "+f"(d[29]), "+f"(d[30]), "+f"(d[31]), "+f"(d[32]), "+f"(d[33]), "+f"(d[34]), "+f"(d[35]), "+f"(d[36]), "+f"(d[37]), "+f"(d[38]), "+f"(d[39]), "+f"(d[40]), "+f"(d[41]), "+f"(d[42]), "+f"(d[43]), "+f"(d[44]), "+f"(d[45]), "+f"(d[46]), "+f"(d[47]), "+f"(d[48]), "+f"(d[49]), "+f"(d[50]), "+f"(d[51]), "+f"(d[52]), "+f"(d[53]), "+f"(d[54]), "+f"(d[55]), "+f"(d[56]), "+f"(d[57]), "+f"(d[58]), "+f"(d[59]), "+f"(d[60]), "+f"(d[61]), "+f"(d[62]), "+f"(d[63]), "+f"(d[64]), "+f"(d[65]), "+f"(d[66]), "+f"(d[67]), "+f"(d[68]), "+f"(d[69]), "+f"(d[70]), "+f"(d[71])
+      : "r"(a[0]), "r"(a[1]), "r"(a[2]), "r"(a[3]), "l"(db), "r"(scale_d));
+}
+template <>
+__device__ __forceinline__ void wgmma_rs_tb<160>(float* d, const uint32_t* a, uint64_t db, uint32_t scale_d) {
+  asm volatile(
+      "{\n\t.reg .pred p;\n\tsetp.ne.b32 p, %85, 0;\n\t"
+      "wgmma.mma_async.sync.aligned.m64n160k16.f32.f16.f16 {%0, %1, %2, %3, %4, %5, %6, %7, %8, %9, %10, %11, %12, %13, %14, %15, %16, %17, %18, %19, %20, %21, %22, %23, %24, %25, %26, %27, %28, %29, %30, %31, %32, %33, %34, %35, %36, %37, %38, %39, %40, %41, %42, %43, %44, %45, %46, %47, %48, %49, %50, %51, %52, %53, %54, %55, %56, %57, %58, %59, %60, %61, %62, %63, %64, %65, %66, %67, %68, %69, %70, %71, %72, %73, %74, %75, %76, %77, %78, %79}, {%80, %81, %82, %83}, %84, p, 1, 1, 1;\n\t}\n"
+      : "+f"(d[0]), "+f"(d[1]), "+f"(d[2]), "+f"(d[3]), "+f"(d[4]), "+f"(d[5]), "+f"(d[6]), "+f"(d[7]), "+f"(d[8]), "+f"(d[9]), "+f"(d[10]), "+f"(d[11]), "+f"(d[12]), "+f"(d[13]), "+f"(d[14]), "+f"(d[15]), "+f"(d[16]), "+f"(d[17]), "+f"(d[18]), "+f"(d[19]), "+f"(d[20]), "+f"(d[21]), "+f"(d[22]), "+f"(d[23]), "+f"(d[24]), "+f"(d[25]), "+f"(d[26]), "+f"(d[27]), "+f"(d[28]), "+f"(d[29]), "+f"(d[30]), "+f"(d[31]), "+f"(d[32]), "+f"(d[33]), "+f"(d[34]), "+f"(d[35]), "+f"(d[36]), "+f"(d[37]), "+f"(d[38]), "+f"(d[39]), "+f"(d[40]), "+f"(d[41]), "+f"(d[42]), "+f"(d[43]), "+f"(d[44]), "+f"(d[45]), "+f"(d[46]), "+f"(d[47]), "+f"(d[48]), "+f"(d[49]), "+f"(d[50]), "+f"(d[51]), "+f"(d[52]), "+f"(d[53]), "+f"(d[54]), "+f"(d[55]), "+f"(d[56]), "+f"(d[57]), "+f"(d[58]), "+f"(d[59]), "+f"(d[60]), "+f"(d[61]), "+f"(d[62]), "+f"(d[63]), "+f"(d[64]), "+f"(d[65]), "+f"(d[66]), "+f"(d[67]), "+f"(d[68]), "+f"(d[69]), "+f"(d[70]), "+f"(d[71]), "+f"(d[72]), "+f"(d[73]), "+f"(d[74]), "+f"(d[75]), "+f"(d[76]), "+f"(d[77]), "+f"(d[78]), "+f"(d[79])
+      : "r"(a[0]), "r"(a[1]), "r"(a[2]), "r"(a[3]), "l"(db), "r"(scale_d));
+}
+template <>
+__device__ __forceinline__ void wgmma_rs_tb<176>(float* d, const uint32_t* a, uint64_t db, uint32_t scale_d) {
+  asm volatile(
+      "{\n\t.reg .pred p;\n\tsetp.ne.b32 p, %93, 0;\n\t"
+      "wgmma.mma_async.sync.aligned.m64n176k16.f32.f16.f16 {%0, %1, %2, %3, %4, %5, %6, %7, %8, %9, %10, %11, %12, %13, %14, %15, %16, %17, %18, %19, %20, %21, %22, %23, %24, %25, %26, %27, %28, %29, %30, %31, %32, %33, %34, %35, %36, %37, %38, %39, %40, %41, %42, %43, %44, %45, %46, %47, %48, %49, %50, %51, %52, %53, %54, %55, %56, %57, %58, %59, %60, %61, %62, %63, %64, %65, %66, %67, %68, %69, %70, %71, %72, %73, %74, %75, %76, %77, %78, %79, %80, %81, %82, %83, %84, %85, %86, %87}, {%88, %89, %90, %91}, %92, p, 1, 1, 1;\n\t}\n"
+      : "+f"(d[0]), "+f"(d[1]), "+f"(d[2]), "+f"(d[3]), "+f"(d[4]), "+f"(d[5]), "+f"(d[6]), "+f"(d[7]), "+f"(d[8]), "+f"(d[9]), "+f"(d[10]), "+f"(d[11]), "+f"(d[12]), "+f"(d[13]), "+f"(d[14]), "+f"(d[15]), "+f"(d[16]), "+f"(d[17]), "+f"(d[18]), "+f"(d[19]), "+f"(d[20]), "+f"(d[21]), "+f"(d[22]), "+f"(d[23]), "+f"(d[24]), "+f"(d[25]), "+f"(d[26]), "+f"(d[27]), "+f"(d[28]), "+f"(d[29]), "+f"(d[30]), "+f"(d[31]), "+f"(d[32]), "+f"(d[33]), "+f"(d[34]), "+f"(d[35]), "+f"(d[36]), "+f"(d[37]), "+f"(d[38]), "+f"(d[39]), "+f"(d[40]), "+f"(d[41]), "+f"(d[42]), "+f"(d[43]), "+f"(d[44]), "+f"(d[45]), "+f"(d[46]), "+f"(d[47]), "+f"(d[48]), "+f"(d[49]), "+f"(d[50]), "+f"(d[51]), "+f"(d[52]), "+f"(d[53]), "+f"(d[54]), "+f"(d[55]), "+f"(d[56]), "+f"(d[57]), "+f"(d[58]), "+f"(d[59]), "+f"(d[60]), "+f"(d[61]), "+f"(d[62]), "+f"(d[63]), "+f"(d[64]), "+f"(d[65]), "+f"(d[66]), "+f"(d[67]), "+f"(d[68]), "+f"(d[69]), "+f"(d[70]), "+f"(d[71]), "+f"(d[72]), "+f"(d[73]), "+f"(d[74]), "+f"(d[75]), "+f"(d[76]), "+f"(d[77]), "+f"(d[78]), "+f"(d[79]), "+f"(d[80]), "+f"(d[81]), "+f"(d[82]), "+f"(d[83]), "+f"(d[84]), "+f"(d[85]), "+f"(d[86]), "+f"(d[87])
       : "r"(a[0]), "r"(a[1]), "r"(a[2]), "r"(a[3]), "l"(db), "r"(scale_d));
 }
 template <>
```
